# lipku/LiveTalking

Hardware: AMD Instinct MI355X
Metric: inferfps (higher is better)
Workload: dtype f16; 1 GPU; wav2lip256, 1 session(s)/GPU, 16-frame batch, fp16 activations / fp32 accumulate, through LipReal.inference_batch; sessions_per_gpu=1, batch=16, parallelism=session-sharded x1 (no collective)

## Files before the change

### livetalking_amd/csrc/conv3_mfma.hip

```cpp
#include "conv_host.h"
#include "misc_kernels.h"
#include "tune.h"

#include <hip/hip_fp16.h>
#include <stdio.h>
#include <stdlib.h>
#include <string.h>

#include <algorithm>
#include <type_traits>
#include <vector>

#ifndef LTK_ABLATE_BUILD
#define LTK_ABLATE_BUILD 0
#endif

namespace ltk {

#if LTK_ABLATE_BUILD
#define ABL(a, bit) ((a).ablate & (bit))
#else
#define ABL(a, bit) 0
#endif

// ... 149 lines not shown
        }
    };

    constexpr int DXN = ((T == 9 && G == 1) || (G == 4 && T == 16)) ? 3 : (G == 4 ? 2 : 1);
    int aj[PXW][DXN];
#pragma unroll
    for (int j = 0; j < PXW; ++j) {
        const int m = (wave * PXW + j) * 32 + l31;
        const int tx = m & TWm;
        const int ty = (m >> a.log2TW) & THm;
        const int b = m >> (a.log2TW + a.log2TH);
        const bool in = b < a.NB;
        const int prow = in ? (b * a.PH + ty * S) * a.PW : 0;
        const int pcol = in ? tx * S : 0;
#pragma unroll
        for (int dx = 0; dx < DXN; ++dx) {
            if constexpr (S == 2) {
                const int pc = pcol + dx;
                const int q = (2 * (pc & 1) + hh) ^ ((pc >> 3) & 3);
                aj[j][dx] = (prow + ((pc & ~1) | (q >> 1))) * 32 + ((q & 1) << 4);
            } else {
                const int key = (a.swz_x & ((pcol + dx) >> 3) & 1) ^ (a.swz_row & (in ? b * a.PH + ty * S : 0) & 1);
                aj[j][dx] = (prow + pcol + dx) * 32 + ((key ^ (Q == 2 ? 0 : hh)) << 4);
            }
        }
    }

    f32x16 acc[G][NBT][PXW];
#pragma unroll
    for (int g = 0; g < G; ++g)
#pragma unroll
        for (int i = 0; i < NBT; ++i)
#pragma unroll
            for (int j = 0; j < PXW; ++j)
#pragma unroll
                for (int r = 0; r < 16; ++r) acc[g][i][j][r] = 0.f;

    const int PS = a.SLOTS * 16;
    const int rowB = a.PW * 32;
    const int rowflip = (S == 1) ? (a.swz_row << 4) : 0;
    auto arow = [&](int v, int dy) -> int { return (dy & 1) ? (v ^ rowflip) : v; };
    auto compute = [&](int buf) {
        const unsigned char* Ab = smem + buf * STAGE;
        const unsigned char* Bb = Ab + A_BYTES;
#pragma unroll
        for (int j = 0; j < PXW; ++j)
#pragma unroll
            for (int dx = 0; dx < DXN; ++dx) asm volatile("" : "+v"(aj[j][dx]));
        if constexpr (Q == 2) {
            const unsigned char* Ap = Ab + hh * PS;
            i32x8 xa[2][PXW], wf[2][NBT];
            auto load_tap = [&](int t, int sl) {
                const unsigned char* Ar = Ap + (t / 3) * rowB;
#pragma unroll
                for (int i = 0; i < NBT; ++i) {
                    const i32x4 lo = *reinterpret_cast<const i32x4*>(Bb + ((((i * T + t) * NC8 + 2 * hh) * 32) + l31) * 16);
                    const i32x4 hi = *reinterpret_cast<const i32x4*>(Bb + ((((i * T + t) * NC8 + 2 * hh + 1) * 32) + l31) * 16);
                    wf[sl][i] = (i32x8){lo[0], lo[1], lo[2], lo[3], hi[0], hi[1], hi[2], hi[3]};
                }
#pragma unroll
                for (int j = 0; j < PXW; ++j) {
                    const i32x4 lo = *reinterpret_cast<const i32x4*>(Ar + arow(aj[j][t % 3], t / 3));
                    const i32x4 hi = *reinterpret_cast<const i32x4*>(Ar + (arow(aj[j][t % 3], t / 3) ^ 16));
                    xa[sl][j] = (i32x8){lo[0], lo[1], lo[2], lo[3], hi[0], hi[1], hi[2], hi[3]};
                }
            };
            load_tap(0, 0);
            __builtin_amdgcn_sched_group_barrier(0x100, 2 * (NBT + PXW), 0);
#pragma unroll
            for (int t = 0; t < T; ++t) {
                const int sl = t & 1;
                if (t + 1 < T) load_tap(t + 1, sl ^ 1);
#pragma unroll
                for (int i = 0; i < NBT; ++i)
#pragma unroll
                    for (int j = 0; j < PXW; ++j)
                        acc[0][i][j] = __builtin_amdgcn_mfma_scale_f32_32x32x64_f8f6f4(wf[sl][i], xa[sl][j], acc[0][i][j], 0, 0, 0, 0x7f7f7f7f, 0,
                                                                                       0x7f7f7f7f);
                if (t + 1 < T) {
                    __builtin_amdgcn_sched_group_barrier(0x100, 2 * (NBT + PXW), 0);
                    __builtin_amdgcn_sched_group_barrier(0x008, NBT * PXW, 0);
                }
            }
        } else
#pragma unroll
        for (int q = 0; q < NCB; ++q) {
            const int plane = 2 * q + hh;
            const unsigned char* Ap = Ab + q * PS;
            if constexpr (G == 1) {
                f16x8 xa[2][PXW], wf[2][NBT];
                auto load_tap = [&](int t, int sl) {
                    const unsigned char* Ar = Ap + ((T == 9) ? (t / 3) * rowB : 0);
#pragma unroll
                    for (int i = 0; i < NBT; ++i)
                        wf[sl][i] = *reinterpret_cast<const f16x8*>(Bb + ((((i * T + t) * NC8 + plane) * 32) + l31) * 16);
#pragma unroll
                    for (int j = 0; j < PXW; ++j) xa[sl][j] = *reinterpret_cast<const f16x8*>(Ar + arow(aj[j][(T == 9) ? t % 3 : 0], (T == 9) ? t / 3 : 0));
                };
                load_tap(0, 0);
                if (T > 1) __builtin_amdgcn_sched_group_barrier(0x100, NBT + PXW, 0);
#pragma unroll
                for (int t = 0; t < T; ++t) {
                    const int sl = t & 1;
                    if (t + 1 < T) load_tap(t + 1, sl ^ 1);
#pragma unroll
                    for (int i = 0; i < NBT; ++i)
#pragma unroll
                        for (int j = 0; j < PXW; ++j) {
                            if constexpr (Q == 0) {
                                acc[0][i][j] = __builtin_amdgcn_mfma_f32_32x32x16_f16(wf[sl][i], xa[sl][j], acc[0][i][j], 0, 0, 0);
                            } else {
                                const i64x2 wq = __builtin_bit_cast(i64x2, wf[sl][i]);
                                const i64x2 xq = __builtin_bit_cast(i64x2, xa[sl][j]);
                                acc[0][i][j] = __builtin_amdgcn_mfma_f32_32x32x16_fp8_fp8(wq[0], xq[0], acc[0][i][j], 0, 0, 0);
                                acc[0][i][j] = __builtin_amdgcn_mfma_f32_32x32x16_fp8_fp8(wq[1], xq[1], acc[0][i][j], 0, 0, 0);
                            }
                        }
                    if (t + 1 < T) {
                        __builtin_amdgcn_sched_group_barrier(0x100, NBT + PXW, 0);
                        __builtin_amdgcn_sched_group_barrier(0x008, NBT * PXW * MPP, 0);
                    }
                }
            } else if constexpr (T == 16) {
                auto wfrag = [&](int t) {
                    return *reinterpret_cast<const f16x8*>(Bb + (((t * NC8 + plane) * 32) + l31) * 16);
                };
                int t = 0;
#pragma unroll
                for (int dy = 0; dy < 3; ++dy)
#pragma unroll
                    for (int dx = 0; dx < 3; ++dx) {
                        f16x8 xa[PXW];
#pragma unroll
                        for (int j = 0; j < PXW; ++j) xa[j] = *reinterpret_cast<const f16x8*>(Ap + dy * rowB + arow(aj[j][dx], dy));
#pragma unroll
                        for (int py = 0; py < 2; ++py)
#pragma unroll
                            for (int px = 0; px < 2; ++px) {
                                if ((dy != py && dy != py + 1) || (dx != px && dx != px + 1)) continue;
                                const f16x8 wf = wfrag(t++);
#pragma unroll
                                for (int j = 0; j < PXW; ++j)
                                    acc[py * 2 + px][0][j] = __builtin_amdgcn_mfma_f32_32x32x16_f16(wf, xa[j], acc[py * 2 + px][0][j], 0, 0, 0);
                            }
                    }
            } else {
                auto wfrag = [&](int t) {
                    return *reinterpret_cast<const f16x8*>(Bb + (((t * NC8 + plane) * 32) + l31) * 16);
                };
                f16x8 xa[PXW];
#pragma unroll
                for (int j = 0; j < PXW; ++j) xa[j] = *reinterpret_cast<const f16x8*>(Ap + aj[j][0]);
#pragma unroll
                for (int t = 0; t < 4; ++t) {
                    const f16x8 wf = wfrag(t);
#pragma unroll
                    for (int j = 0; j < PXW; ++j)
                        acc[t][0][j] = __builtin_amdgcn_mfma_f32_32x32x16_f16(wf, xa[j], acc[t][0][j], 0, 0, 0);
                }
#pragma unroll
                for (int j = 0; j < PXW; ++j) xa[j] = *reinterpret_cast<const f16x8*>(Ap + aj[j][G == 4 ? 1 : 0]);
                {
                    const f16x8 w4 = wfrag(4), w5 = wfrag(5);
#pragma unroll
                    for (int j = 0; j < PXW; ++j) {
                        acc[1][0][j] = __builtin_amdgcn_mfma_f32_32x32x16_f16(w4, xa[j], acc[1][0][j], 0, 0, 0);
                        acc[3][0][j] = __builtin_amdgcn_mfma_f32_32x32x16_f16(w5, xa[j], acc[3][0][j], 0, 0, 0);
                    }
                }
#pragma unroll
                for (int j = 0; j < PXW; ++j) xa[j] = *reinterpret_cast<const f16x8*>(Ap + rowB + arow(aj[j][0], 1));
                {
                    const f16x8 w6 = wfrag(6), w7 = wfrag(7);
#pragma unroll
                    for (int j = 0; j < PXW; ++j) {
                        acc[2][0][j] = __builtin_amdgcn_mfma_f32_32x32x16_f16(w6, xa[j], acc[2][0][j], 0, 0, 0);
                        acc[3][0][j] = __builtin_amdgcn_mfma_f32_32x32x16_f16(w7, xa[j], acc[3][0][j], 0, 0, 0);
                    }
                }
#pragma unroll
                for (int j = 0; j < PXW; ++j) xa[j] = *reinterpret_cast<const f16x8*>(Ap + rowB + arow(aj[j][G == 4 ? 1 : 0], 1));
                {
                    const f16x8 w8 = wfrag(8);
#pragma unroll
                    for (int j = 0; j < PXW; ++j)
                        acc[3][0][j] = __builtin_amdgcn_mfma_f32_32x32x16_f16(w8, xa[j], acc[3][0][j], 0, 0, 0);
                }
            }
        }
    };

    __syncthreads();
    stage(c_begin, 0);
    if (T != 1 && wave < 2 && lane < BN / 4)
        GLDS16((wave ? a.shift : a.scale) + ntile * BN + lane * 4, smem + a.lds_scale_off + wave * (BN * 4));
    for (int c = c_begin; c < c_end; ++c) {
        const int cur = (c - c_begin) & 1;
        __syncthreads();
        if (c + 1 < c_end) stage(c + 1, cur ^ 1);
        if (!ABL(a, 4)) compute(cur);
    }

#if LTK_ABLATE_BUILD
    if (a.ablate & 64) return;
    if (a.ablate & 128) {
        float t = 0.f;
#pragma unroll
        for (int g = 0; g < G; ++g)
#pragma unroll
            for (int i = 0; i < NBT; ++i)
#pragma unroll
                for (int j = 0; j < PXW; ++j) t += acc[g][i][j][0] + acc[g][i][j][7];
        if (t == 12345.678f) a.y[0] = (f16)t;
        return;
    }
#endif
    const int cout0 = ntile * BN;
    const int HWo = a.HoA * a.WoA;
    int l31_e = l31;
    asm volatile("" : "+v"(l31_e));
    auto out_px = [&](int j, int g, int* n_out, bool* ok) -> int {
        const int m = (wave * PXW + j) * 32 + l31_e;
        const int tx = m & TWm;
        const int ty = (m >> a.log2TW) & THm;
        const int b = m >> (a.log2TW + a.log2TH);
        const int n = n0 + b, y = ty0 + ty, x = tx0 + tx;
        *ok = (b < a.NB) && (n < a.N) && (y < a.Ho) && (x < a.Wo);
        *n_out = n;
        const int oy = (G == 4) ? 2 * y + (g >> 1) : y;
        const int ox = (G == 4) ? 2 * x + (g & 1) : x;
        return oy * a.WoA + ox;
    };

    if constexpr (HEAD) {
        const float* const sb = reinterpret_cast<const float*>(smem + a.lds_scale_off);
        float p[PXW][3];
#pragma unroll
        for (int j = 0; j < PXW; ++j) p[j][0] = p[j][1] = p[j][2] = 0.f;
#pragma unroll
        for (int q4 = 0; q4 < 4; ++q4) {
            const int cl = 8 * q4 + 4 * hh;
            const f32x4 sc = *reinterpret_cast<const f32x4*>(sb + cl), sf = *reinterpret_cast<const f32x4*>(sb + 32 + cl);
            const f32x4 w0 = *reinterpret_cast<const f32x4*>(hd->w + cl), w1 = *reinterpret_cast<const f32x4*>(hd->w + 32 + cl),
                        w2 = *reinterpret_cast<const f32x4*>(hd->w + 64 + cl);
#pragma unroll
            for (int j = 0; j < PXW; ++j)
#pragma unroll
                for (int r = 0; r < 4; ++r) {
                    const float v = __builtin_amdgcn_fmed3f(acc[0][0][j][4 * q4 + r] * sc[r] + sf[r], 0.f, 65504.f);
                    p[j][0] += v * w0[r]; p[j][1] += v * w1[r]; p[j][2] += v * w2[r];
                }
        }
        const float b0 = hd->w[96], b1 = hd->w[97], b2 = hd->w[98];
#pragma unroll
        for (int j = 0; j < PXW; ++j) {
            bool ok;
            int n;
            const int opx = out_px(j, 0, &n, &ok);
            const float t0 = p[j][0] + __shfl_xor(p[j][0], 32), t1 = p[j][1] + __shfl_xor(p[j][1], 32),
                        t2 = p[j][2] + __shfl_xor(p[j][2], 32);
            const float s0 = 1.f / (1.f + __expf(-(t0 + b0)));
            const float s1 = 1.f / (1.f + __expf(-(t1 + b1)));
            const float s2 = 1.f / (1.f + __expf(-(t2 + b2)));
            unsigned char* const o = ok ? hd->outs->p[n] : nullptr;
            if (o && hh == 0) {
                unsigned char* q = o + (size_t)opx * 3;
                q[0] = (unsigned char)(unsigned)(s0 * 255.f);
                q[1] = (unsigned char)(unsigned)(s1 * 255.f);
                q[2] = (unsigned char)(unsigned)(s2 * 255.f);
            }
// ... 159 lines not shown
            const int cbo2 = cout0 >> 5;
            int obase[PXW];
            bool okj[PXW];
            float lmean[PXW], lrstd[PXW];
            const bool ln_cons = a.ln_in != nullptr;
#pragma unroll
            for (int j = 0; j < PXW; ++j) {
                int n;
                const int opx = out_px(j, 0, &n, &okj[j]);
                obase[j] = ((n * a.y_cbt + a.y_cb0 + cbo2) * HWo + opx) * 16 + hh * 8;
                lmean[j] = 0.f; lrstd[j] = 1.f;
                if (ln_cons) ln_token_stats(okj[j] ? n * HWo + opx : 0, &lmean[j], &lrstd[j]);
            }
#pragma unroll
            for (int i = 0; i < NBT; ++i) {
                if (2 * i >= ncb_valid) continue;
                f32x4 scv[2], sfv[2], scg[2], sfg[2];
#pragma unroll
                for (int eo = 0; eo < 2; ++eo) {
                    const int cl = cout0 + i * 32 + 8 * eo + 4 * hh;
                    scv[eo] = *reinterpret_cast<const f32x4*>(a.scale + cl);      sfv[eo] = *reinterpret_cast<const f32x4*>(a.shift + cl);
                    scg[eo] = *reinterpret_cast<const f32x4*>(a.scale + cl + 16); sfg[eo] = *reinterpret_cast<const f32x4*>(a.shift + cl + 16);
                }
#pragma unroll
                for (int j = 0; j < PXW; ++j) {
                    unsigned pk[2][2];
#pragma unroll
                    for (int eo = 0; eo < 2; ++eo) {
                        f16x4 o;
#pragma unroll
                        for (int r = 0; r < 4; ++r) {
                            float v, gt;
                            if (ln_cons) {
                                v = lrstd[j] * (acc[0][i][j][4 * eo + r] - lmean[j] * scv[eo][r]) + sfv[eo][r];
                                gt = lrstd[j] * (acc[0][i][j][4 * (2 + eo) + r] - lmean[j] * scg[eo][r]) + sfg[eo][r];
                            } else {
                                v = acc[0][i][j][4 * eo + r] * scv[eo][r] + sfv[eo][r];
                                gt = acc[0][i][j][4 * (2 + eo) + r] * scg[eo][r] + sfg[eo][r];
                            }
                            const float t = v * gelu_as(gt);
                            o[r] = (f16)__builtin_amdgcn_fmed3f(t, -65504.f, 65504.f);
                        }
                        const uint2 u = *reinterpret_cast<const uint2*>(&o);
                        pk[eo][0] = u.x; pk[eo][1] = u.y;
                    }
                    const auto s0 = __builtin_amdgcn_permlane32_swap(pk[0][0], pk[1][0], false, false);
                    const auto s1 = __builtin_amdgcn_permlane32_swap(pk[0][1], pk[1][1], false, false);
                    const uint4 out = make_uint4(s0[0], s1[0], s0[1], s1[1]);
                    if (okj[j] && do_store) *reinterpret_cast<uint4*>(a.y + obase[j] + i * HWo16) = out;
                }
            }
            return;
        }
    }
    if (a.relu == 1) epilogue(std::integral_constant<int, 1>{});
    else if (a.relu == 2) epilogue(std::integral_constant<int, 2>{});
    else if (a.relu == 3) epilogue(std::integral_constant<int, 3>{});
    else epilogue(std::integral_constant<int, 0>{});
}

template <int G, int NBT, int PXW, int NC8, int T, int S = 1, int Q = 0>
__global__ __launch_bounds__(256, 2) void conv3_kernel(const K3Args a) {
    extern __shared__ __attribute__((aligned(16))) unsigned char smem[];
    const int nblk = gridDim.x;
    const int q = nblk >> 3, r = nblk & 7;
    const int xcd = blockIdx.x & 7, slot = blockIdx.x >> 3;
    const int first = (xcd < r ? xcd * (q + 1) : r * (q + 1) + (xcd - r) * q) + slot;
    for (int item = first; item < a.nitems; item += nblk) {
        if (item != first) __syncthreads();
        conv3_item<G, NBT, PXW, NC8, T, S, Q>(a, item, smem);
    }
}

template <int PXW>
__global__ __launch_bounds__(256, 2) void conv3_head_kernel(const K3Args a, const HeadArgs h) {
    extern __shared__ __attribute__((aligned(16))) unsigned char smem[];
    const int nblk = gridDim.x;
    const int q = nblk >> 3, r = nblk & 7;
    const int xcd = blockIdx.x & 7, slot = blockIdx.x >> 3;
    const int first = (xcd < r ? xcd * (q + 1) : r * (q + 1) + (xcd - r) * q) + slot;
    for (int item = first; item < a.nitems; item += nblk) {
        if (item != first) __syncthreads();
        conv3_item<1, 1, PXW, 2, 9, 1, 0, 1>(a, item, smem, &h);
    }
}

__global__ __launch_bounds__(256) void conv3_finish_kernel(const float* __restrict__ partial, int ksplit, long long Mtot, int HWo,
                                                            int CoutP, int Cout, const float* __restrict__ scale,
                                                            const float* __restrict__ shift, const f16* __restrict__ res,
                                                            int res_cbt, int res_cb0, f16* __restrict__ y, int y_cbt, int y_cb0,
                                                            int relu) {
    const int ncb = Cout >> 4;
    const long long i = (long long)blockIdx.x * 256 + threadIdx.x;
    if (i >= Mtot * ncb * 2) return;
    const int half = (int)(i & 1);
    const long long r2 = i >> 1;
    const long long row = r2 % Mtot;
    const int cb = (int)(r2 / Mtot);
    const int n = (int)(row / HWo), opx = (int)(row - (long long)n * HWo);
    const int c0 = cb * 16 + half * 8;
    float v[8];
#pragma unroll
    for (int r = 0; r < 8; ++r) v[r] = 0.f;
    for (int s = 0; s < ksplit; ++s) {
        const float* p = partial + ((size_t)s * Mtot + row) * CoutP + c0;
        const f32x4 a0 = *reinterpret_cast<const f32x4*>(p), a1 = *reinterpret_cast<const f32x4*>(p + 4);
#pragma unroll
        for (int r = 0; r < 4; ++r) { v[r] += a0[r]; v[4 + r] += a1[r]; }
    }
    f16x8 rr;
    if (res) rr = *reinterpret_cast<const f16x8*>(res + (((size_t)n * res_cbt + res_cb0 + cb) * HWo + opx) * 16 + half * 8);
    f16x8 o;
#pragma unroll
    for (int r = 0; r < 8; ++r) {
        float t = v[r] * scale[c0 + r] + shift[c0 + r];
        if (res) t += (float)rr[r];
        if (relu == 1) t = fmaxf(t, 0.f);
        else if (relu >= 2) t = (relu == 2) ? 0.5f * t * (1.f + erff(t * 0.70710678118654752f)) : t / (1.f + __expf(-t));
        t = fminf(fmaxf(t, -65504.f), 65504.f);
        o[r] = (f16)t;
    }
    *reinterpret_cast<f16x8*>(y + (((size_t)n * y_cbt + y_cb0 + cb) * HWo + opx) * 16 + half * 8) = o;
}


template <int KB, int KPB, int KS>
__global__ __launch_bounds__(256 * KS, KS == 1 ? 2 : 1) void lin_fk_kernel(const K3Args a, const int cpg, const int ngroups, const int nslabs) {
    extern __shared__ __attribute__((aligned(16))) unsigned char smem[];
    const int tid = threadIdx.x;
    const int lane = tid & 63;
    const int wave8 = __builtin_amdgcn_readfirstlane(tid >> 6);
    const int wave = wave8 & 3, kh = wave8 >> 2;
    const int l31 = lane & 31, hh = lane >> 5;
    const int grp = blockIdx.x % ngroups, mt = blockIdx.x / ngroups;
    const int s_begin = grp * cpg, s_end = min(nslabs, s_begin + cpg);
    const int P = a.HoA * a.WoA;
    constexpr int SLAB = KB * KS * 1024;
    constexpr int PXW = 1;
    constexpr int KP = KB / KPB;
    constexpr int PART = KPB * 1024;
    constexpr int STAGE = KS * PART;
    constexpr int SS_OFF = 2 * STAGE;
    constexpr int XCH_OFF = SS_OFF + 512;
    static_assert(KB % KPB == 0 && KPB % 4 == 0 && (KS == 1 || KS == 2), "whole parts, whole KiB pieces per wave");
    bool ok[PXW];
    int n[PXW], pix[PXW];
#pragma unroll
    for (int j = 0; j < PXW; ++j) {
        const long long m = (long long)mt * (128 * PXW) + (wave * PXW + j) * 32 + l31;
        ok[j] = m < a.Mtot;
        const int mm = (int)(ok[j] ? m : a.Mtot - 1);
        n[j] = mm / P; pix[j] = mm - n[j] * P;
    }

    const unsigned char* const wbase = reinterpret_cast<const unsigned char*>(a.w);
    auto stage = [&](int s, int h, int buf) {
        const unsigned char* src = wbase + (size_t)s * SLAB + (kh * KP + h) * PART + lane * 16;
        unsigned char* dst = smem + buf * STAGE + kh * PART;
#pragma unroll
        for (int k = 0; k < KPB / 4; ++k) GLDS16(src + (k * 4 + wave) * 1024, dst + (k * 4 + wave) * 1024);
        if (h == 0 && wave8 == 0 && lane < 16)
            GLDS16((lane < 8 ? a.scale : a.shift - 32) + s * 32 + lane * 4, smem + SS_OFF + ((s - s_begin) & 1) * 256);
    };
    stage(s_begin, 0, 0);
    int parts_done = 0;

// ... 410 lines not shown
    K3M(2, 2); K3M(1, 2); K3M(2, 1); K3M(1, 1);
#undef K3M
    return nullptr;
}

static k3_kernel_t k3_pick_s2(int NBT, int NC8) {
    return k3_pick_f16(1, NBT, 2, NC8, 9, 2);
}

constexpr int kMaxKSplit = 32;

bool conv3_lin_fk_k(int Cin) { return Cin == 320 || Cin == 640 || Cin == 512 || Cin == 384 || Cin == 1280; }

int conv3_lin_mp_nsl(int Cin, long long rows, int Cout) {
    const int kn = knob(K_LIN_MP);
    if (!kn || !knob(K_LIN_FK) || !(Cin == 2560 || Cin == 5120) || rows < kLinFkMinRows || Cout % 16) return 0;
    if (kn == 2 || kn == 3) return kn;
    const long long mt = (rows + 127) / 128;
    const int nslabs = (Cout + 31) / 32;
    for (int nsl = 2; nsl <= 3; ++nsl)
        if (mt * ((nslabs + nsl - 1) / nsl) <= 256) return nsl;
    return 0;
}

static int k3_ksplit(long long base, int nchunks, int cap) {
    if (nchunks < 4) return 1;
    int s;
    if (cap > 0) {
        if (base >= 128) {
            if (!(cap == 4 && nchunks >= 60 && base <= 1024)) return 1;
            s = 4;
        } else {
            s = std::min(cap, (int)((256 + base - 1) / base));
        }
    } else {
        if (base >= 200 || (base >= 128 && nchunks < 48)) return 1;
        s = (int)((256 + base - 1) / base);
    }
    s = std::min(s, std::min(nchunks / 2, kMaxKSplit));
    return std::max(s, 1);
}

size_t conv3_partial_bytes(const ConvPlan& p, int N, int H, int W) {
    if (!p.v3) return 0;
    int Ho = H, Wo = W;
    if (p.v3_G == 4) { Ho = 2 * H; Wo = 2 * W; }
    return (size_t)kMaxKSplit * N * Ho * Wo * p.CoutPad * sizeof(float);
}

struct K3Tile {
    int l2w, l2h, NB;
    int PH, PW, npix, SLOTS;
    int swz_x, swz_row;
    int tiles_x, tiles_y, tiles_n;
    long long blocks;
    bool fit;
};

static K3Tile k3_tile(int pxw, int N, int Ho, int Wo, int S, int ext, int NC8, int T) {
    K3Tile t;
    const int M = 128 * pxw;
    const int lm = ceil_log2(M);
    t.l2w = std::min(5, ceil_log2(Wo));
    t.l2h = std::min(lm - t.l2w, ceil_log2(Ho));
    t.NB = M >> (t.l2w + t.l2h);
    t.NB = std::max(1, std::min(t.NB, N));
    t.PH = ((1 << t.l2h) - 1) * S + 1 + ext; t.PW = ((1 << t.l2w) - 1) * S + 1 + ext;
    if (S == 2) t.PW = (t.PW + 1) & ~1;
    t.swz_x = 1; t.swz_row = 0;
    if (S == 1 && t.l2w <= 4) {
        t.swz_x = 0; t.swz_row = 1;
        if (t.l2w == 3 && ext > 0) t.PW = 12;
    }
    while (t.NB > 1 && (NC8 / 2) * ((2 * t.NB * t.PH * t.PW + 63) / 64 * 64) > k3_maxa(pxw, NC8, S, T) * 256) --t.NB;
    t.npix = t.NB * t.PH * t.PW;
    t.SLOTS = (2 * t.npix + 63) / 64 * 64;
    t.tiles_x = (Wo + (1 << t.l2w) - 1) >> t.l2w; t.tiles_y = (Ho + (1 << t.l2h) - 1) >> t.l2h;
    t.tiles_n = (N + t.NB - 1) / t.NB;
    t.blocks = (long long)t.tiles_x * t.tiles_y * t.tiles_n;
    t.fit = (NC8 / 2) * t.SLOTS <= k3_maxa(pxw, NC8, S, T) * 256 && t.npix < 32768;
    return t;
}

static K3Tile k3_choose_tile(const ConvPlan& p, int N, int Ho, int Wo, int ext, int nchunks, int kn_pxw, int kn_nbt, bool forced_tile, bool head,
                             int* PXW, int* NBT) {
    const int G = p.v3_G, T = p.v3_T, NC8 = p.NC8, S = p.v3_S;
    if (G == 1 && T == 9 && S == 1 && kn_pxw == 0 && kn_nbt == 0) {
        static const int cand[6][2] = {{4, 2}, {4, 1}, {2, 2}, {2, 1}, {1, 2}, {1, 1}};
        K3Tile best = {};
        for (int ci = 0; ci < 6; ++ci) {
            const int pxw = cand[ci][0], nbt = cand[ci][1];
            if ((pxw == 4 && NC8 != 2) || (nbt == 2 && p.lCout < 64) || (pxw == 4 && nbt == 1 && p.lCout >= 64)) continue;
            if (head && pxw == 1) continue;
            const K3Tile t = k3_tile(pxw, N, Ho, Wo, S, ext, NC8, T);
            if (!t.fit) continue;
            best = t; *PXW = pxw; *NBT = nbt;
            if (t.blocks * ((p.lCout + 32 * nbt - 1) / (32 * nbt)) >= (nchunks >= 40 ? 256 : 384)) break;
        }
        return best;
    }
    K3Tile t = k3_tile(*PXW, N, Ho, Wo, S, ext, NC8, T);
    if (*PXW == 4) {
        const long long nt = (p.lCout + 32 * *NBT - 1) / (32 * *NBT);
        constexpr int kPxw4MinItems = 448;
        if (!t.fit || (!forced_tile && t.blocks * nt < kPxw4MinItems)) { *PXW = 2; t = k3_tile(*PXW, N, Ho, Wo, S, ext, NC8, T); }
    }
    return t;
}

struct K3Launch {
    enum Family { CONV3, HEAD, LIN } family;
    const void* kernel;
    unsigned grid, block;
    size_t lds;
    int lds_attr;
    int lin[3];
    K3Args a;
};

int conv3_plan_launch(const ConvPlan& p, const ConvIO& io_in, K3Launch* k3, std::string* err) {
    K3Launch local;
    K3Launch& L = k3 ? *k3 : local;
    ConvIO io = io_in;
    if (p.ups4) {
        if (!io.ups || ((io.H | io.W) & 1)) { if (err) *err = "conv3: a four-phase upsample-conv plan needs ups = 1 and even H, W"; return -1; }
        io.H /= 2; io.W /= 2; io.ups = 0;
    }
    K3Args& a = L.a;
    memset(&a, 0, sizeof(a));
    const int G = p.v3_G, T = p.v3_T, NC8 = p.NC8;
    a.N = io.N; a.H = io.H; a.W = io.W; a.x_cbt = io.x_ld >> 4; a.x_cb0 = io.x_coff >> 4;
    a.res_cbt = io.res_ld >> 4; a.res_cb0 = io.res_coff >> 4;
    int y_ld = io.y_ld;
    a.relu = io.relu ? 1 : io.act;
    a.ups = io.ups ? 1 : 0;
    if (io.ups && ((io.H | io.W) & 1)) { if (err) *err = "conv3: upsampled input needs even H, W"; return -1; }
    a.Cout = p.lCout; a.CoutP = p.CoutPad;
    int ext;
    const int S = p.v3_S;
    a.Ho = io.H; a.Wo = io.W;
    if (G == 4) { a.HoA = 2 * io.H; a.WoA = 2 * io.W; a.pad = p.ups4 ? 1 : 0; ext = p.ups4 ? 2 : 1; }
    else if (S == 2) {
        a.Ho = (io.H + 2 * p.ph + p.out_pad - 3) / 2 + 1; a.Wo = (io.W + 2 * p.pw + p.out_pad - 3) / 2 + 1;
        a.HoA = a.Ho; a.WoA = a.Wo; a.pad = p.ph; ext = 2;
    }
    else { a.HoA = io.H; a.WoA = io.W; a.pad = (T == 9) ? 1 : 0; ext = (T == 9) ? 2 : 0; }
    if (p.gemm_1x1_expand) {
        if (io.H != 1 || io.W != 1) { if (err) *err = "k x k transposed conv only supported on 1x1 maps"; return -1; }
        if (io.y_ld != p.Cout || io.y_coff != 0) { if (err) *err = "1x1-expand output must be contiguous"; return -1; }
        y_ld = p.lCout;
    }
    a.y_cbt = y_ld >> 4; a.y_cb0 = io.y_coff >> 4;
    if ((io.x_ld | io.x_coff | y_ld | io.y_coff | p.lCout) & 15) { if (err) *err = "conv3: channel counts/offsets must be multiples of 16"; return -1; }
    if (io.res && ((io.res_ld | io.res_coff) & 15)) { if (err) *err = "conv3: residual channel count/offset must be a multiple of 16"; return -1; }
    if ((double)io.N * io.H * io.W * io.x_ld >= 2147483647.0 || (double)io.N * a.HoA * a.WoA >= 2147483647.0) {
        if (err) *err = "tensor too large for 32-bit offsets"; return -1;
    }
    a.nchunks = (p.Cin / 8) / NC8;
    a.Mtot = (long long)io.N * a.HoA * a.WoA;
    const bool head = io.head_w != nullptr && io.head_outs != nullptr;

    int NBT = (G == 4) ? 1 : ((p.lCout >= 64) ? 2 : 1);
    int PXW = (G == 1 && T == 9 && NC8 == 2 && S == 1) ? 4 : 2;
    const int kn_pxw = io.force_pxw ? io.force_pxw : knob(K_CONV_PXW), kn_nbt = io.force_nbt ? io.force_nbt : knob(K_CONV3_NBT);
    if (kn_pxw == 2 || (kn_pxw == 1 && G == 1 && T == 9 && S == 1) || (kn_pxw == 4 && PXW == 4)) PXW = kn_pxw;
    if (kn_nbt == 1) NBT = 1;
    const bool forced_tile = io.force_pxw != 0 && io.force_nbt != 0;
    const bool conv3x3 = G == 1 && T == 9 && S == 1;
    const K3Tile tile = k3_choose_tile(p, io.N, a.Ho, a.Wo, ext, a.nchunks, kn_pxw, kn_nbt, forced_tile, head, &PXW, &NBT);
    if (!tile.fit) { if (err) *err = "conv3: patch does not fit the staging budget"; return -1; }
    const long long blocks = tile.blocks;
    a.tiles_x = tile.tiles_x; a.tiles_y = tile.tiles_y; a.tiles_n = tile.tiles_n;
    if (T == 1 && NC8 == 4 && G == 1 && p.lCout % 128 == 0 && ((blocks * (p.lCout / 128) >= 384 && kn_nbt == 0) || kn_nbt == 4)) NBT = 4;
    if (NBT == 2 && blocks * ((p.lCout + 63) / 64) < ((T == 1 && blocks >= 4) ? 256 : 128) && !conv3x3 && !forced_tile) NBT = 1;
    if (io.report && ((io.force_pxw && PXW != io.force_pxw) || (io.force_nbt && NBT != io.force_nbt))) {
        if (err) *err = "conv3: no kernel instantiation for the forced tile (pxw " + std::to_string(io.force_pxw) + ", nbt " + std::to_string(io.force_nbt) +
                        "): this layer takes pxw " + std::to_string(PXW) + ", nbt " + std::to_string(NBT);
        return -1;
    }
    const int BN = NBT * 32;
    a.n_ntiles = (p.lCout + BN - 1) / BN;
    a.ablate = LTK_ABLATE_BUILD ? knob(K_ABLATE) : 0;

    int ksplit = knob(K_SPLITK) ? k3_ksplit(blocks * a.n_ntiles, a.nchunks, T == 1 ? 0 : (G == 4 ? 8 : 4)) : 1;
    const int fks = io.force_ksplit ? io.force_ksplit : knob(K_KSPLIT);
    if (fks > 0 && knob(K_SPLITK)) ksplit = std::max(1, std::min(std::min(fks, kMaxKSplit), a.nchunks));
    if (head) ksplit = 1;
    a.ln_out_tiles = io.ln_out_tiles; a.ln_in_tiles = io.ln_in_tiles; a.ln_eps = io.ln_eps;
    if (io.ln_out || io.ln_in) {
        if (!(G == 1 && T == 1 && !p.q8) || (io.ln_out && (p.lCout % 32 || io.ln_out_tiles != p.lCout / 32)) || (io.ln_in && io.ln_in_tiles <= 0)) {
            if (err) *err = "conv3: the LayerNorm fold is a 1x1-layer feature (32-channel tiles)"; return -1;
        }
        ksplit = 1;
    }
    if (a.relu == 4) {
        if (!(G == 1 && T == 1 && !p.q8 && p.lCout % 32 == 0 && !io.res)) { if (err) *err = "conv3: the GEGLU epilogue is a 1x1-layer feature"; return -1; }
        ksplit = 1;
    }

    const int mp_nsl = (G == 1 && T == 1 && S == 1) ? conv3_lin_mp_nsl(p.Cin, a.Mtot, p.lCout) : 0;
    if (G == 1 && T == 1 && S == 1 && !p.q8 && !p.mx && !a.ups && !p.gemm_1x1_expand && knob(K_LIN_FK) && (conv3_lin_fk_k(p.Cin) || mp_nsl) &&
        a.nchunks * NC8 * 8 == p.Cin && a.Mtot >= kLinFkMinRows && a.ablate == 0 && p.lCout % 16 == 0 &&
        (a.relu == 0 || a.relu == 1 || a.relu == 4)) {
        typedef void (*lin_t)(const K3Args, int, int, int);
        const int nslabs = (p.lCout + 31) / 32;
        const long long mtiles = (a.Mtot + 127) / 128;
        L.family = K3Launch::LIN;
        a.ksplit = 1;
        if (mp_nsl) {
            const int NSL = mp_nsl;
            const int ng = (nslabs + NSL - 1) / NSL;
            L.kernel = (const void*)(NSL == 2 ? (lin_t)lin_mp_kernel<2> : (lin_t)lin_mp_kernel<3>);
            L.lds = (size_t)2 * 2 * 20 * 1024 + 1024 + (size_t)NSL * 4 * 4096;
            L.lds_attr = (int)L.lds;
            L.grid = (unsigned)(mtiles * ng); L.block = 512;
            L.lin[0] = ng; L.lin[1] = nslabs; L.lin[2] = p.Cin / 1280;
            if (io.report) { *io.report = ConvReport(); snprintf(io.report->kernel, sizeof(io.report->kernel), "lin_mp_kernel<%d>", NSL); }
            return 0;
        }
        constexpr int kLinFkBlocks = 512;
        const int want = p.Cin == 1280 ? kLinFkBlocks / 2 : kLinFkBlocks;
        int ngroups = (int)std::max(1ll, std::min((long long)nslabs, (want + mtiles - 1) / mtiles));
        const int cpg = (nslabs + ngroups - 1) / ngroups;
        ngroups = (nslabs + cpg - 1) / cpg;
        const long long grid = mtiles * ngroups;
        if (grid > 0 && grid <= 0x7fffffffll) {
            const lin_t lk = p.Cin == 320 ? (lin_t)lin_fk_kernel<20, 20, 1> : p.Cin == 640 ? (lin_t)lin_fk_kernel<40, 20, 1> : p.Cin == 512 ? (lin_t)lin_fk_kernel<32, 16, 1>
                           : p.Cin == 384 ? (lin_t)lin_fk_kernel<24, 24, 1> : (lin_t)lin_fk_kernel<40, 20, 2>;
            const int ks = p.Cin == 1280 ? 2 : 1;
            L.kernel = (const void*)lk;
            L.lds = (size_t)2 * ks * (p.Cin == 512 ? 16 : p.Cin == 384 ? 24 : 20) * 1024 + 512 + (ks == 2 ? 2 * 4 * 4096 : 0);
            L.lds_attr = (int)L.lds;
            L.grid = (unsigned)grid; L.block = 256 * ks;
            L.lin[0] = cpg; L.lin[1] = ngroups; L.lin[2] = nslabs;
            if (io.report) { *io.report = ConvReport(); snprintf(io.report->kernel, sizeof(io.report->kernel), "lin_fk_kernel"); }
            return 0;
        }
    }

    if (ksplit > 1) {
        while (ksplit > 1 && (!io.partial || io.partial_cap < (size_t)ksplit * a.Mtot * p.CoutPad * sizeof(float))) ksplit /= 2;
    }
    a.ksplit = ksplit;
    a.chunks_per_split = (a.nchunks + ksplit - 1) / ksplit;
    if ((long long)a.chunks_per_split * (ksplit - 1) >= a.nchunks) {
        ksplit = (a.nchunks + a.chunks_per_split - 1) / a.chunks_per_split;
        a.ksplit = ksplit;
    }
    a.log2TW = tile.l2w; a.log2TH = tile.l2h; a.NB = tile.NB; a.PH = tile.PH; a.PW = tile.PW; a.npix = tile.npix; a.SLOTS = tile.SLOTS;
    a.swz_x = tile.swz_x; a.swz_row = tile.swz_row;
    a.magicPW = magic_u16(tile.PW); a.magicPHW = magic_u16(tile.PH * tile.PW);

    const size_t a_bytes = (size_t)(NC8 / 2) * a.SLOTS * 16, b_bytes = (size_t)T * NC8 * BN * 16;
    size_t lds = 2 * (a_bytes + b_bytes);
    lds = (lds + 255) / 256 * 256;
    a.lds_scale_off = (int)lds;
    if (T != 1) lds += 2 * BN * sizeof(float);
    if (lds > 160 * 1024) { if (err) *err = "conv3: LDS budget exceeded"; return -1; }

    if (p.q8 && !(G == 1 && T == 9 && S == 1)) { if (err) *err = "conv3: fp8 operands are implemented for 3x3 stride-1 convs"; return -1; }
    if (head && !(G == 1 && T == 9 && S == 1 && !p.q8 && NC8 == 2 && NBT == 1 && p.lCout == 32 && (PXW == 4 || PXW == 2) && ksplit == 1)) {
        if (err) *err = "conv3: fused head needs the 3x3 stride-1 32-cout configuration";
        return -1;
    }
    k3_kernel_t k = p.mx ? k3_pick_mx(NBT, PXW) : p.q8 ? k3_pick_q8(NBT, PXW, NC8) : (S == 2) ? k3_pick_s2(NBT, NC8) : k3_pick(G, NBT, PXW, NC8, T);
    if (!k) { if (err) *err = "conv3: no kernel instantiation"; return -1; }
    const long long nblk = blocks * a.n_ntiles * ksplit;
    if (nblk <= 0 || nblk > 0x7fffffffll) { if (err) *err = "bad grid"; return -1; }
    a.nitems = (int)nblk;
    constexpr int kPersistBlocks = 512;
    const long long grid = nblk > kPersistBlocks ? kPersistBlocks : nblk;
    L.family = head ? K3Launch::HEAD : K3Launch::CONV3;
    L.kernel = (const void*)k;
    if (head) {
        typedef void (*k3_head_t)(const K3Args, const HeadArgs);
        L.kernel = (const void*)(PXW == 4 ? (k3_head_t)conv3_head_kernel<4> : (k3_head_t)conv3_head_kernel<2>);
    }
    L.grid = (unsigned)grid; L.block = 256; L.lds = lds; L.lds_attr = 160 * 1024;
    if (io.report) {
        ConvReport& r = *io.report;
        r = ConvReport();
        const std::string nm = head ? "conv3_head_kernel<" + std::to_string(PXW) + ">" : p.mx ? "conv3_kernel (mx)" : p.q8 ? "conv3_kernel (fp8)" : k3_name(G, NBT, PXW, NC8, T, S);
        snprintf(r.kernel, sizeof(r.kernel), "%s", nm.c_str());
        r.G = G; r.NBT = NBT; r.PXW = PXW; r.NC8 = NC8; r.T = T; r.S = S; r.ksplit = ksplit; r.items = (int)nblk; r.grid = (int)grid;
    }
    return 0;
}

int conv3_launch(const ConvPlan& p, const ConvIO& io, hipStream_t stream, std::string* err) {
    K3Launch L;
    if (const int rc = conv3_plan_launch(p, io, &L, err)) return rc;
    K3Args& a = L.a;
    a.x = io.x; a.w = p.d_w; a.scale = p.d_scale; a.shift = p.d_shift; a.res = io.res; a.y = io.y;
    a.ln_out = io.ln_out; a.ln_in = io.ln_in;
    a.partial = a.ksplit > 1 ? io.partial : nullptr;
    HIPCHK((hipError_t)ensure_dyn_lds(L.kernel, L.lds_attr));
    switch (L.family) {
    case K3Launch::LIN:
        hipLaunchKernelGGL((void (*)(const K3Args, int, int, int))L.kernel, dim3(L.grid), dim3(L.block), L.lds, stream, a, L.lin[0], L.lin[1], L.lin[2]);
        break;
    case K3Launch::HEAD: {
        HeadArgs h;
        h.w = io.head_w;
        h.outs = reinterpret_cast<const OutPtrs*>(io.head_outs);
        hipLaunchKernelGGL((void (*)(const K3Args, const HeadArgs))L.kernel, dim3(L.grid), dim3(L.block), L.lds, stream, a, h);
        break;
    }
    case K3Launch::CONV3:
        hipLaunchKernelGGL((k3_kernel_t)L.kernel, dim3(L.grid), dim3(L.block), L.lds, stream, a);
        break;
    }
    HIPCHK(hipGetLastError());
    if (a.ksplit > 1) {
        const long long items = a.Mtot * (p.lCout >> 3);
        hipLaunchKernelGGL(conv3_finish_kernel, dim3((unsigned)((items + 255) / 256)), dim3(256), 0, stream,
                           (const float*)io.partial, a.ksplit, a.Mtot, a.HoA * a.WoA, p.CoutPad, p.lCout, (const float*)p.d_scale,
                           (const float*)p.d_shift, io.res, a.res_cbt, a.res_cb0, io.y, a.y_cbt, a.y_cb0, a.relu);
        HIPCHK(hipGetLastError());
    }
    return 0;
}

}
```

### livetalking_amd/csrc/w2l_program.hip

```cpp
#include "engine_internal.h"

namespace {

struct LayerDef {
    const char* prefix;
    bool transposed;
    int cin, cout, k, sh, sw, pad, out_pad;
    bool residual;
};

const LayerDef kAudio[] = {
    {"audio_encoder.0", false, 1, 32, 3, 1, 1, 1, 0, false},
    {"audio_encoder.1", false, 32, 32, 3, 1, 1, 1, 0, true},
    {"audio_encoder.2", false, 32, 32, 3, 1, 1, 1, 0, true},
    {"audio_encoder.3", false, 32, 64, 3, 3, 1, 1, 0, false},
    {"audio_encoder.4", false, 64, 64, 3, 1, 1, 1, 0, true},
    {"audio_encoder.5", false, 64, 64, 3, 1, 1, 1, 0, true},
    {"audio_encoder.6", false, 64, 128, 3, 3, 3, 1, 0, false},
    {"audio_encoder.7", false, 128, 128, 3, 1, 1, 1, 0, true},
    {"audio_encoder.8", false, 128, 128, 3, 1, 1, 1, 0, true},
    {"audio_encoder.9", false, 128, 256, 3, 3, 2, 1, 0, false},
    {"audio_encoder.10", false, 256, 256, 3, 1, 1, 1, 0, true},
    {"audio_encoder.11", false, 256, 512, 3, 1, 1, 0, 0, false},
    {"audio_encoder.12", false, 512, 512, 1, 1, 1, 0, 0, false},
};
struct BlockLayer { int block; LayerDef d; };
const BlockLayer kFaceEnc[] = {
    {0, {"face_encoder_blocks.0.0", false, 6, 16, 7, 1, 1, 3, 0, false}},
    {1, {"face_encoder_blocks.1.0", false, 16, 32, 3, 2, 2, 1, 0, false}},
    {1, {"face_encoder_blocks.1.1", false, 32, 32, 3, 1, 1, 1, 0, true}},
    {1, {"face_encoder_blocks.1.2", false, 32, 32, 3, 1, 1, 1, 0, true}},
    {2, {"face_encoder_blocks.2.0", false, 32, 64, 3, 2, 2, 1, 0, false}},
    {2, {"face_encoder_blocks.2.1", false, 64, 64, 3, 1, 1, 1, 0, true}},
    {2, {"face_encoder_blocks.2.2", false, 64, 64, 3, 1, 1, 1, 0, true}},
    {2, {"face_encoder_blocks.2.3", false, 64, 64, 3, 1, 1, 1, 0, true}},
    {3, {"face_encoder_blocks.3.0", false, 64, 128, 3, 2, 2, 1, 0, false}},
    {3, {"face_encoder_blocks.3.1", false, 128, 128, 3, 1, 1, 1, 0, true}},
    {3, {"face_encoder_blocks.3.2", false, 128, 128, 3, 1, 1, 1, 0, true}},
    {4, {"face_encoder_blocks.4.0", false, 128, 256, 3, 2, 2, 1, 0, false}},
    {4, {"face_encoder_blocks.4.1", false, 256, 256, 3, 1, 1, 1, 0, true}},
    {4, {"face_encoder_blocks.4.2", false, 256, 256, 3, 1, 1, 1, 0, true}},
    {5, {"face_encoder_blocks.5.0", false, 256, 512, 3, 2, 2, 1, 0, false}},
    {5, {"face_encoder_blocks.5.1", false, 512, 512, 3, 1, 1, 1, 0, true}},
    {6, {"face_encoder_blocks.6.0", false, 512, 512, 3, 2, 2, 1, 0, false}},
    {6, {"face_encoder_blocks.6.1", false, 512, 512, 3, 1, 1, 1, 0, true}},
    {7, {"face_encoder_blocks.7.0", false, 512, 512, 4, 1, 1, 0, 0, false}},
    {7, {"face_encoder_blocks.7.1", false, 512, 512, 1, 1, 1, 0, 0, false}},
};
const BlockLayer kFaceDec[] = {
    {0, {"face_decoder_blocks.0.0", false, 512, 512, 1, 1, 1, 0, 0, false}},
    {1, {"face_decoder_blocks.1.0", true, 1024, 512, 4, 1, 1, 0, 0, false}},
    {1, {"face_decoder_blocks.1.1", false, 512, 512, 3, 1, 1, 1, 0, true}},
    {2, {"face_decoder_blocks.2.0", true, 1024, 512, 3, 2, 2, 1, 1, false}},
    {2, {"face_decoder_blocks.2.1", false, 512, 512, 3, 1, 1, 1, 0, true}},
    {3, {"face_decoder_blocks.3.0", true, 1024, 512, 3, 2, 2, 1, 1, false}},
    {3, {"face_decoder_blocks.3.1", false, 512, 512, 3, 1, 1, 1, 0, true}},
    {3, {"face_decoder_blocks.3.2", false, 512, 512, 3, 1, 1, 1, 0, true}},
    {4, {"face_decoder_blocks.4.0", true, 768, 384, 3, 2, 2, 1, 1, false}},
    {4, {"face_decoder_blocks.4.1", false, 384, 384, 3, 1, 1, 1, 0, true}},
    {4, {"face_decoder_blocks.4.2", false, 384, 384, 3, 1, 1, 1, 0, true}},
    {5, {"face_decoder_blocks.5.0", true, 512, 256, 3, 2, 2, 1, 1, false}},
    {5, {"face_decoder_blocks.5.1", false, 256, 256, 3, 1, 1, 1, 0, true}},
    {5, {"face_decoder_blocks.5.2", false, 256, 256, 3, 1, 1, 1, 0, true}},
    {6, {"face_decoder_blocks.6.0", true, 320, 128, 3, 2, 2, 1, 1, false}},
    {6, {"face_decoder_blocks.6.1", false, 128, 128, 3, 1, 1, 1, 0, true}},
    {6, {"face_decoder_blocks.6.2", false, 128, 128, 3, 1, 1, 1, 0, true}},
    {7, {"face_decoder_blocks.7.0", true, 160, 64, 3, 2, 2, 1, 1, false}},
    {7, {"face_decoder_blocks.7.1", false, 64, 64, 3, 1, 1, 1, 0, true}},
    {7, {"face_decoder_blocks.7.2", false, 64, 64, 3, 1, 1, 1, 0, true}},
};
const LayerDef kOutConv = {"output_block.0", false, 80, 32, 3, 1, 1, 1, 0, false};
const float kBnEps = 1e-5f;

int frame_bucket(int nf) { return nf <= 16 ? 0 : nf <= 32 ? 1 : nf <= 64 ? 2 : nf <= 128 ? 3 : 4; }

struct TileEntry { const char* layer; int bucket, pxw, nbt, ks; };
const TileEntry kTileTable[] = {
    {"face_encoder_blocks.5.1", 0, 2, 1, 0},
    {"face_decoder_blocks.2.1", 0, 2, 1, 0},
    {"face_encoder_blocks.6.0", 0, 0, 0, 8},
    {"face_decoder_blocks.1.0", 0, 0, 0, 4},
    {"audio_encoder.7", 0, 0, 0, 1},
    {"audio_encoder.8", 0, 0, 0, 1},
    {"face_decoder_blocks.4.1", 2, 2, 2, 0},
    {"face_decoder_blocks.4.2", 2, 2, 2, 0},
    {"face_encoder_blocks.5.0", 2, 2, 1, 0},
    {"face_encoder_blocks.6.1", 2, 1, 2, 0},
    {"face_decoder_blocks.1.1", 2, 1, 2, 0},
    {"face_decoder_blocks.1.0", 2, 0, 0, 4},
};

int check_tile_table_impl(std::string& msg) {
    int bad = 0;
    auto find = [](const char* name) -> const LayerDef* {
        for (const LayerDef& d : kAudio) if (!strcmp(d.prefix, name)) return &d;
        for (const BlockLayer& b : kFaceEnc) if (!strcmp(b.d.prefix, name)) return &b.d;
        for (const BlockLayer& b : kFaceDec) if (!strcmp(b.d.prefix, name)) return &b.d;
        if (!strcmp(kOutConv.prefix, name)) return &kOutConv;
        return nullptr;
    };
    const size_t n = sizeof(kTileTable) / sizeof(kTileTable[0]);
    for (size_t i = 0; i < n; ++i) {
        const TileEntry& t = kTileTable[i];
        auto complain = [&](const char* what) { ++bad; msg += std::string(t.layer) + " (bucket " + std::to_string(t.bucket) + "): " + what + "; "; };
        const LayerDef* d = find(t.layer);
        if (!d) { complain("no such layer"); continue; }
        if (t.bucket < 0 || t.bucket >= 5) complain("bucket outside 0..4");
        if ((t.pxw == 0) != (t.nbt == 0)) complain("pxw and nbt must be given together");
        if (t.pxw != 0 && t.pxw != 1 && t.pxw != 2 && t.pxw != 4) complain("pxw must be 0, 1, 2 or 4");
        if (t.nbt < 0 || t.nbt > 2) complain("nbt must be 0, 1 or 2");
        if (t.ks < 0 || t.ks > 32) complain("split factor outside 0..32");
        if (t.pxw == 0 && t.nbt == 0 && t.ks == 0) complain("entry changes nothing");
        const bool s1_3x3 = !d->transposed && d->k == 3 && d->sh == 1 && d->sw == 1;
        if ((t.pxw == 1 || t.pxw == 4) && !s1_3x3) complain("128- / 512-pixel tiles exist for 3x3 stride-1 layers only");
        if (t.pxw == 4 && d->cout > 32) complain("512-pixel tiles exist for <= 32 output channels only");
        if (t.nbt == 2 && d->cout < 64) complain("64-cout blocks need >= 64 output channels");
        if (d->k == 7) complain("the first layer runs on conv7, not conv3");
        for (size_t j = 0; j < i; ++j)
            if (!strcmp(kTileTable[j].layer, t.layer) && kTileTable[j].bucket == t.bucket) complain("duplicate entry");
    }
    return bad;
}

void apply_tile_table_impl(std::vector<Layer>& layers) {
    for (const TileEntry& t : kTileTable)
        for (Layer& L : layers)
            if (L.name == t.layer) { L.tile[t.bucket].pxw = (signed char)t.pxw; L.tile[t.bucket].nbt = (signed char)t.nbt; L.tile[t.bucket].ks = (signed char)t.ks; }
}


int build_layer_impl(ltk_engine* e, const LayerDef& d, const ltk_named_tensor* sd, int n, Layer* L, int hint_hw, int flat_ld, int map_w) {
    const std::string p = d.prefix;
    const size_t wcount = (size_t)d.cin * d.cout * d.k * d.k;
    SD dict{sd, n, ""};
    const float* w = dict.get(p + ".conv_block.0.weight", wcount);
    const float* b = dict.get(p + ".conv_block.0.bias", d.cout);
    const float* g = dict.get(p + ".conv_block.1.weight", d.cout);
    const float* beta = dict.get(p + ".conv_block.1.bias", d.cout);
    const float* mean = dict.get(p + ".conv_block.1.running_mean", d.cout);
    const float* var = dict.get(p + ".conv_block.1.running_var", d.cout);
    if (!w || !b || !g || !beta || !mean || !var)
        return fail(LTK_E_INVALID, "state_dict is missing (or has a wrong shape for) tensors of layer " + p);
    std::vector<float> sc(d.cout), sf(d.cout);
    fold_bn(g, beta, mean, var, b, kBnEps, d.cout, sc.data(), sf.data());
    std::string err;
    int rc;
    std::vector<float> wfold;
    L->res_folded = false;
    if (d.residual && !d.transposed && d.cin == d.cout && (d.k & 1) && d.sh == 1 && d.sw == 1 && d.pad == d.k / 2) {
        bool ok = true;
        for (int c = 0; c < d.cout; ++c) ok = ok && fabsf(sc[c]) >= 1e-3f;
        if (ok) {
            wfold.assign(w, w + wcount);
            const int kk = d.k * d.k, ctr = (d.k / 2) * d.k + d.k / 2;
            for (int c = 0; c < d.cout; ++c) wfold[((size_t)c * d.cin + c) * kk + ctr] += 1.0f / sc[c];
            w = wfold.data();
            L->res_folded = true;
        }
    }
    if (flat_ld > 0) {
        const int kk = d.k * d.k;
        const int cin_flat = kk * d.cin;
        std::vector<float> wf((size_t)d.cout * cin_flat, 0.f);
        for (int co = 0; co < d.cout; ++co)
            for (int ci = 0; ci < d.cin; ++ci)
                for (int t = 0; t < kk; ++t)
                    wf[(size_t)co * cin_flat + ((size_t)(ci >> 4) * kk + t) * 16 + (ci & 15)] = w[((size_t)co * d.cin + ci) * kk + t];
        rc = conv_plan_create(&L->plan, wf.data(), cin_flat, d.cout, 1, 1, 1, 1, 0, 0, false, 0, sc.data(), sf.data(), &err);
    } else {
        rc = conv_plan_create(&L->plan, w, d.cin, d.cout, d.k, d.k, d.sh, d.sw, d.pad, d.pad, d.transposed, d.out_pad,
                              sc.data(), sf.data(), &err);
    }
    if (rc) return conv_status(rc, p + ": " + err);
    const bool want_rowgemm = knob(K_ROWGEMM) && knob(K_SPLITK), want_rowconv = knob(K_ROWCONV) > 0 && knob(K_SPLITK);
    {
        std::vector<float> we, se, fe;
        int J = 0, K = 0;
        if (flat_ld > 0) {
            const int kk = d.k * d.k;
            J = d.cout; K = kk * d.cin;
            we.assign((size_t)J * K, 0.f);
            for (int co = 0; co < d.cout; ++co)
                for (int ci = 0; ci < d.cin; ++ci)
                    for (int t = 0; t < kk; ++t)
                        we[(size_t)co * K + ((size_t)(ci >> 4) * kk + t) * 16 + (ci & 15)] = w[((size_t)co * d.cin + ci) * kk + t];
            se = sc; fe = sf;
        } else if (!d.transposed && d.k == 1 && hint_hw == 1 && d.cin % 32 == 0 && d.cout % 16 == 0) {
            J = d.cout; K = d.cin;
            we.assign(w, w + (size_t)J * K);
            se = sc; fe = sf;
        } else if (d.transposed && hint_hw == 1 && d.sh == 1 && d.pad == 0 && d.out_pad == 0 && d.cin % 32 == 0 && d.cout % 16 == 0) {
            const int kk = d.k * d.k;
            J = kk * d.cout; K = d.cin;
            we.assign((size_t)J * K, 0.f); se.assign(J, 0.f); fe.assign(J, 0.f);
            for (int j = 0; j < J; ++j) {
                const int c16 = j & 15, tt = j >> 4, pos = tt % kk, co = (tt / kk) * 16 + c16;
                for (int ci = 0; ci < d.cin; ++ci) we[(size_t)j * K + ci] = w[((size_t)ci * d.cout + co) * kk + pos];
// ... 400 lines not shown
```

Baseline: 13680 frames/s.

## Add software-pipelined 128-pixel tile kernel for stride-2 transposed 3x3 convs

Adds a dedicated G==4/T==9 compute path for transposed 3x3 stride-2 convolutions. It double-buffers weight and activation fragment loads across sub-pixel phase steps and uses sched_group_barrier so MFMA work overlaps the loads. It also adds a conv3t_px128_kernel instantiation with 128-pixel tiles and a heuristic that picks the smaller tile when the 256-pixel tiling yields too few work items. Tile-table entries route two decoder layers to this path, one with a split-K factor. The cost is extra register pressure from double buffering, plus a new kernel variant that must be validated for those layers.

```diff
diff --git a/livetalking_amd/csrc/conv3_mfma.hip b/livetalking_amd/csrc/conv3_mfma.hip
--- a/livetalking_amd/csrc/conv3_mfma.hip
+++ b/livetalking_amd/csrc/conv3_mfma.hip
@@ -255,6 +255,44 @@
                     __builtin_amdgcn_sched_group_barrier(0x008, NBT * PXW, 0);
                 }
             }
+        } else if constexpr (G == 4 && T == 9) {
+            constexpr int NS = NCB * 4;
+            f16x8 xa[2][PXW], wf[2][4];
+            auto nw = [](int o) { return o == 0 ? 4 : o == 3 ? 1 : 2; };
+            auto load_step = [&](int s, int sl) {
+                const int qq = s >> 2, o = s & 3, t0 = o == 0 ? 0 : 2 + 2 * o;
+                const unsigned char* Ar = Ab + qq * PS + (o >> 1) * rowB;
+#pragma unroll
+                for (int w = 0; w < nw(o); ++w)
+                    wf[sl][w] = *reinterpret_cast<const f16x8*>(Bb + ((((t0 + w) * NC8 + 2 * qq + hh) * 32) + l31) * 16);
+#pragma unroll
+                for (int j = 0; j < PXW; ++j) xa[sl][j] = *reinterpret_cast<const f16x8*>(Ar + arow(aj[j][o & 1], o >> 1));
+            };
+            load_step(0, 0);
+            __builtin_amdgcn_sched_group_barrier(0x100, 4 + PXW, 0);
+            auto step = [&](auto o_tag, const int s) {
+                constexpr int o = decltype(o_tag)::value, sl = o & 1;
+                constexpr int NW = o == 0 ? 4 : o == 3 ? 1 : 2, NWN = o == 3 ? 4 : o == 2 ? 1 : 2;
+                if (s + 1 < NS) load_step(s + 1, sl ^ 1);
+#pragma unroll
+                for (int w = 0; w < NW; ++w) {
+                    const int g = o == 0 ? w : o == 1 ? 1 + 2 * w : o == 2 ? 2 + w : 3;
+#pragma unroll
+                    for (int j = 0; j < PXW; ++j)
+                        acc[g][0][j] = __builtin_amdgcn_mfma_f32_32x32x16_f16(wf[sl][w], xa[sl][j], acc[g][0][j], 0, 0, 0);
+                }
+                if (s + 1 < NS) {
+                    __builtin_amdgcn_sched_group_barrier(0x100, NWN + PXW, 0);
+                    __builtin_amdgcn_sched_group_barrier(0x008, NW * PXW, 0);
+                }
+            };
+#pragma unroll
+            for (int qq = 0; qq < NCB; ++qq) {
+                step(std::integral_constant<int, 0>{}, 4 * qq);
+                step(std::integral_constant<int, 1>{}, 4 * qq + 1);
+                step(std::integral_constant<int, 2>{}, 4 * qq + 2);
+                step(std::integral_constant<int, 3>{}, 4 * qq + 3);
+            }
         } else
 #pragma unroll
         for (int q = 0; q < NCB; ++q) {
@@ -294,7 +332,7 @@
                         __builtin_amdgcn_sched_group_barrier(0x008, NBT * PXW * MPP, 0);
                     }
                 }
-            } else if constexpr (T == 16) {
+            } else {
                 auto wfrag = [&](int t) {
                     return *reinterpret_cast<const f16x8*>(Bb + (((t * NC8 + plane) * 32) + l31) * 16);
                 };
@@ -317,48 +355,6 @@
                                     acc[py * 2 + px][0][j] = __builtin_amdgcn_mfma_f32_32x32x16_f16(wf, xa[j], acc[py * 2 + px][0][j], 0, 0, 0);
                             }
                     }
-            } else {
-                auto wfrag = [&](int t) {
-                    return *reinterpret_cast<const f16x8*>(Bb + (((t * NC8 + plane) * 32) + l31) * 16);
-                };
-                f16x8 xa[PXW];
-#pragma unroll
-                for (int j = 0; j < PXW; ++j) xa[j] = *reinterpret_cast<const f16x8*>(Ap + aj[j][0]);
-#pragma unroll
-                for (int t = 0; t < 4; ++t) {
-                    const f16x8 wf = wfrag(t);
-#pragma unroll
-                    for (int j = 0; j < PXW; ++j)
-                        acc[t][0][j] = __builtin_amdgcn_mfma_f32_32x32x16_f16(wf, xa[j], acc[t][0][j], 0, 0, 0);
-                }
-#pragma unroll
-                for (int j = 0; j < PXW; ++j) xa[j] = *reinterpret_cast<const f16x8*>(Ap + aj[j][G == 4 ? 1 : 0]);
-                {
-                    const f16x8 w4 = wfrag(4), w5 = wfrag(5);
-#pragma unroll
-                    for (int j = 0; j < PXW; ++j) {
-                        acc[1][0][j] = __builtin_amdgcn_mfma_f32_32x32x16_f16(w4, xa[j], acc[1][0][j], 0, 0, 0);
-                        acc[3][0][j] = __builtin_amdgcn_mfma_f32_32x32x16_f16(w5, xa[j], acc[3][0][j], 0, 0, 0);
-                    }
-                }
-#pragma unroll
-                for (int j = 0; j < PXW; ++j) xa[j] = *reinterpret_cast<const f16x8*>(Ap + rowB + arow(aj[j][0], 1));
-                {
-                    const f16x8 w6 = wfrag(6), w7 = wfrag(7);
-#pragma unroll
-                    for (int j = 0; j < PXW; ++j) {
-                        acc[2][0][j] = __builtin_amdgcn_mfma_f32_32x32x16_f16(w6, xa[j], acc[2][0][j], 0, 0, 0);
-                        acc[3][0][j] = __builtin_amdgcn_mfma_f32_32x32x16_f16(w7, xa[j], acc[3][0][j], 0, 0, 0);
-                    }
-                }
-#pragma unroll
-                for (int j = 0; j < PXW; ++j) xa[j] = *reinterpret_cast<const f16x8*>(Ap + rowB + arow(aj[j][G == 4 ? 1 : 0], 1));
-                {
-                    const f16x8 w8 = wfrag(8);
-#pragma unroll
-                    for (int j = 0; j < PXW; ++j)
-                        acc[3][0][j] = __builtin_amdgcn_mfma_f32_32x32x16_f16(w8, xa[j], acc[3][0][j], 0, 0, 0);
-                }
             }
         }
     };
@@ -684,6 +680,19 @@
     for (int item = first; item < a.nitems; item += nblk) {
         if (item != first) __syncthreads();
         conv3_item<1, 1, PXW, 2, 9, 1, 0, 1>(a, item, smem, &h);
+    }
+}
+
+template <int NC8>
+__global__ __launch_bounds__(256, 3) void conv3t_px128_kernel(const K3Args a) {
+    extern __shared__ __attribute__((aligned(16))) unsigned char smem[];
+    const int nblk = gridDim.x;
+    const int q = nblk >> 3, r = nblk & 7;
+    const int xcd = blockIdx.x & 7, slot = blockIdx.x >> 3;
+    const int first = (xcd < r ? xcd * (q + 1) : r * (q + 1) + (xcd - r) * q) + slot;
+    for (int item = first; item < a.nitems; item += nblk) {
+        if (item != first) __syncthreads();
+        conv3_item<4, 1, 1, NC8, 9, 1, 0>(a, item, smem);
     }
 }
 
@@ -1260,6 +1269,8 @@
     return t;
 }
 
+constexpr int kConvT128BelowItems = 384;
+
 static K3Tile k3_choose_tile(const ConvPlan& p, int N, int Ho, int Wo, int ext, int nchunks, int kn_pxw, int kn_nbt, bool forced_tile, bool head,
                              int* PXW, int* NBT) {
     const int G = p.v3_G, T = p.v3_T, NC8 = p.NC8, S = p.v3_S;
@@ -1276,6 +1287,16 @@
             if (t.blocks * ((p.lCout + 32 * nbt - 1) / (32 * nbt)) >= (nchunks >= 40 ? 256 : 384)) break;
         }
         return best;
+    }
+    if (G == 4 && T == 9 && kn_pxw == 0) {
+        const long long nt = (p.lCout + 31) / 32;
+        const K3Tile t2 = k3_tile(2, N, Ho, Wo, S, ext, NC8, T);
+        if (!t2.fit || t2.blocks * nt < kConvT128BelowItems) {
+            const K3Tile t1 = k3_tile(1, N, Ho, Wo, S, ext, NC8, T);
+            if (t1.fit) { *PXW = 1; return t1; }
+        }
+        *PXW = 2;
+        return t2;
     }
     K3Tile t = k3_tile(*PXW, N, Ho, Wo, S, ext, NC8, T);
     if (*PXW == 4) {
@@ -1341,7 +1362,8 @@
     int NBT = (G == 4) ? 1 : ((p.lCout >= 64) ? 2 : 1);
     int PXW = (G == 1 && T == 9 && NC8 == 2 && S == 1) ? 4 : 2;
     const int kn_pxw = io.force_pxw ? io.force_pxw : knob(K_CONV_PXW), kn_nbt = io.force_nbt ? io.force_nbt : knob(K_CONV3_NBT);
-    if (kn_pxw == 2 || (kn_pxw == 1 && G == 1 && T == 9 && S == 1) || (kn_pxw == 4 && PXW == 4)) PXW = kn_pxw;
+    const bool convT = G == 4 && T == 9;
+    if (kn_pxw == 2 || (kn_pxw == 1 && ((G == 1 && T == 9 && S == 1) || convT)) || (kn_pxw == 4 && PXW == 4)) PXW = kn_pxw;
     if (kn_nbt == 1) NBT = 1;
     const bool forced_tile = io.force_pxw != 0 && io.force_nbt != 0;
     const bool conv3x3 = G == 1 && T == 9 && S == 1;
@@ -1441,7 +1463,9 @@
         if (err) *err = "conv3: fused head needs the 3x3 stride-1 32-cout configuration";
         return -1;
     }
-    k3_kernel_t k = p.mx ? k3_pick_mx(NBT, PXW) : p.q8 ? k3_pick_q8(NBT, PXW, NC8) : (S == 2) ? k3_pick_s2(NBT, NC8) : k3_pick(G, NBT, PXW, NC8, T);
+    const bool t128 = convT && PXW == 1 && NBT == 1 && !p.q8 && !p.mx && (NC8 == 2 || NC8 == 4);
+    k3_kernel_t k = t128 ? (NC8 == 2 ? (k3_kernel_t)conv3t_px128_kernel<2> : (k3_kernel_t)conv3t_px128_kernel<4>)
+                  : p.mx ? k3_pick_mx(NBT, PXW) : p.q8 ? k3_pick_q8(NBT, PXW, NC8) : (S == 2) ? k3_pick_s2(NBT, NC8) : k3_pick(G, NBT, PXW, NC8, T);
     if (!k) { if (err) *err = "conv3: no kernel instantiation"; return -1; }
     const long long nblk = blocks * a.n_ntiles * ksplit;
     if (nblk <= 0 || nblk > 0x7fffffffll) { if (err) *err = "bad grid"; return -1; }
@@ -1458,7 +1482,7 @@
     if (io.report) {
         ConvReport& r = *io.report;
         r = ConvReport();
-        const std::string nm = head ? "conv3_head_kernel<" + std::to_string(PXW) + ">" : p.mx ? "conv3_kernel (mx)" : p.q8 ? "conv3_kernel (fp8)" : k3_name(G, NBT, PXW, NC8, T, S);
+        const std::string nm = head ? "conv3_head_kernel<" + std::to_string(PXW) + ">" : t128 ? "conv3t_px128_kernel<" + std::to_string(NC8) + ">" : p.mx ? "conv3_kernel (mx)" : p.q8 ? "conv3_kernel (fp8)" : k3_name(G, NBT, PXW, NC8, T, S);
         snprintf(r.kernel, sizeof(r.kernel), "%s", nm.c_str());
         r.G = G; r.NBT = NBT; r.PXW = PXW; r.NC8 = NC8; r.T = T; r.S = S; r.ksplit = ksplit; r.items = (int)nblk; r.grid = (int)grid;
     }
diff --git a/livetalking_amd/csrc/w2l_program.hip b/livetalking_amd/csrc/w2l_program.hip
--- a/livetalking_amd/csrc/w2l_program.hip
+++ b/livetalking_amd/csrc/w2l_program.hip
@@ -82,12 +82,14 @@
     {"face_decoder_blocks.1.0", 0, 0, 0, 4},
     {"audio_encoder.7", 0, 0, 0, 1},
     {"audio_encoder.8", 0, 0, 0, 1},
+    {"face_decoder_blocks.3.0", 0, 1, 1, 2},
     {"face_decoder_blocks.4.1", 2, 2, 2, 0},
     {"face_decoder_blocks.4.2", 2, 2, 2, 0},
     {"face_encoder_blocks.5.0", 2, 2, 1, 0},
     {"face_encoder_blocks.6.1", 2, 1, 2, 0},
     {"face_decoder_blocks.1.1", 2, 1, 2, 0},
     {"face_decoder_blocks.1.0", 2, 0, 0, 4},
+    {"face_decoder_blocks.4.0", 2, 1, 1, 0},
 };
 
 int check_tile_table_impl(std::string& msg) {
@@ -112,7 +114,9 @@
         if (t.ks < 0 || t.ks > 32) complain("split factor outside 0..32");
         if (t.pxw == 0 && t.nbt == 0 && t.ks == 0) complain("entry changes nothing");
         const bool s1_3x3 = !d->transposed && d->k == 3 && d->sh == 1 && d->sw == 1;
-        if ((t.pxw == 1 || t.pxw == 4) && !s1_3x3) complain("128- / 512-pixel tiles exist for 3x3 stride-1 layers only");
+        const bool convT3 = d->transposed && d->k == 3 && d->sh == 2 && d->sw == 2;
+        if (t.pxw == 4 && !s1_3x3) complain("512-pixel tiles exist for 3x3 stride-1 layers only");
+        if (t.pxw == 1 && !s1_3x3 && !(convT3 && t.nbt == 1)) complain("128-pixel tiles exist for 3x3 stride-1 layers and, with 32-cout blocks, stride-2 transposed convs only");
         if (t.pxw == 4 && d->cout > 32) complain("512-pixel tiles exist for <= 32 output channels only");
         if (t.nbt == 2 && d->cout < 64) complain("64-cout blocks need >= 64 output channels");
         if (d->k == 7) complain("the first layer runs on conv7, not conv3");
```

Result: no change. 13770 frames/s (median of 6 runs) (+0.7%).
